# rgoldade/GeometricMultigridPressureSolver

Hardware: AMD Instinct MI355X
Metric: V-cycles/sec (higher is better)
Workload: dtype f32

## Files before the change

### geometricmultigridpressuresolver_amd/csrc/mgps_kernels.hip

```cpp
#include <hip/hip_runtime.h>
#include <hip/hip_fp16.h>

#include <algorithm>
#include <cstdlib>
#include <type_traits>

#include "mgps_internal.h"

namespace mgps {

namespace {

typedef float v4f __attribute__((ext_vector_type(4)));
typedef unsigned char v4b __attribute__((ext_vector_type(4)));
__device__ __forceinline__ float4 streamLoad4(const float *p)
{
    const v4f v = __builtin_nontemporal_load(reinterpret_cast<const v4f *>(p));
    return make_float4(v.x, v.y, v.z, v.w);
}
__device__ __forceinline__ uchar4 streamLoad4(const uint8_t *p)
{
    const v4b v = __builtin_nontemporal_load(reinterpret_cast<const v4b *>(p));
    return make_uchar4(v.x, v.y, v.z, v.w);
}
// ... 516 lines not shown
        const float xs[6] = {me[-1], xc.x, xc.y, xc.z, xc.w, me[4]};
        const float yms[4] = {ym.x, ym.y, ym.z, ym.w}, yps[4] = {yp.x, yp.y, yp.z, yp.w};
        const float zms[4] = {xm.x, xm.y, xm.z, xm.w}, zps[4] = {xp.x, xp.y, xp.z, xp.w};
        const float bs[4] = {bc.x, bc.y, bc.z, bc.w};
        const unsigned ls[4] = {lc.x, lc.y, lc.z, lc.w};
        float res[4];
#pragma unroll
        for (int e = 0; e < 4; ++e) {
            const float diag = simpleDiag(ls[e]);
            const float lap = diag * xs[e + 1] - (xs[e] + xs[e + 2] + yms[e] + yps[e] + zms[e] + zps[e]);
            res[e] = simpleCell(ls[e]) ? epilogueRcp<OP_JACOBI>(xs[e + 1], bs[e], lap, simpleRcp(diag), omega) : inactiveValue<OP_JACOBI>(xs[e + 1]);
        }
        if (valid) gStore4nt(scalarBase(out + ptrdiff_t(k) * sz), opq(off), make_float4(res[0], res[1], res[2], res[3]));
        xc = xp;
        xp = xq;
        hy = hyn;
        hx = hxn;
        lc = lcn;
        lcn = lcq;
        buf ^= 1;
    }
}

__global__ __launch_bounds__(64 * kPlaneRows, 8) void residualZKernel(GridP g, float *__restrict__ rz, const float *__restrict__ x,
                                                                     const float *__restrict__ b, unsigned nbx, unsigned nby, int zc,
                                                                     const int32_t *__restrict__ blocks, const float *__restrict__ rEdge)
{
    __shared__ float plane[2][(kPlaneRows + 2) * kPlanePitch];
    unsigned bid = remapBlock(blockIdx.x, gridDim.x);
    if (blocks) bid = unsigned(blocks[bid]);
    bid = __builtin_amdgcn_readfirstlane(bid);
    const unsigned bx = bid % nbx, by = (bid / nbx) % nby, bz = bid / (nbx * nby);
    const int lane = threadIdx.x & (kWave - 1), ty = threadIdx.x / kWave;
    const int i = int(bx) * 256 + lane * 4, j = int(by) * kPlaneRows + ty;
    const int ic = min(i, g.nx - 4), jc = min(j, g.ny - 1);
    const bool live = ic >= g.xlo && ic < g.xhi;
    const bool valid = i < g.nx && j < g.ny && live;
    const size_t sz = size_t(g.nx) * g.ny;
    const int k0 = int(bz) * zc, k1 = min(k0 + zc, g.nz);
    const int ks = max(k0 - 1, 0), ke = min(k1, g.nz - 1);
    const unsigned offL = unsigned(jc) * unsigned(g.nx) + unsigned(min(max(ic, g.xlo), max(g.xhi - 4, g.xlo)));
    const bool rowTop = ty == 0, rowBot = ty == kPlaneRows - 1, colL = lane == 0, colR = lane == kWave - 1;
    const bool hasL = ic > 0, hasR = ic + 4 < g.nx;
    const int kLo = g.ghostLo ? -1 : 0, kHi = g.ghostHi ? g.nz : g.nz - 1;
    auto planeOf = [&](const float *p, int k) { return scalarBase(p + ptrdiff_t(min(max(k, kLo), kHi)) * ptrdiff_t(sz)); };
    float *const mine0 = plane[0] + (ty + 1) * kPlanePitch + 4 + lane * 4;
    constexpr int kBufFloats = (kPlaneRows + 2) * kPlanePitch;
    const unsigned offHy = (rowTop && jc > 0) ? offL - unsigned(g.nx) : (rowBot && jc < g.ny - 1) ? offL + unsigned(g.nx) : offL;
    {
        const float4 xm = gLoad4(planeOf(x, ks - 1), offL);
        *reinterpret_cast<float4 *>(mine0 + kBufFloats) = keepIf(xm, live);
    }
    const float *xk = planeOf(x, ks);
    float4 xc = gLoad4(xk, offL);
    float4 xp = gLoad4(planeOf(x, ks + 1), offL);
    float4 hy = gLoad4(xk, offHy);
    const bool useHx = live && ((colL && hasL) || (colR && hasR));
    const unsigned offHx = !useHx ? offL : colL ? offL - 1u : offL + 4u;
    float hx = gLoad1(xk, offHx);
    constexpr float w0 = 0.125f, w1 = 0.375f, w2 = 0.375f, w3 = 0.125f;
    float accPrev[4] = {0.f, 0.f, 0.f, 0.f}, accCur[4] = {0.f, 0.f, 0.f, 0.f};
    if (rEdge && k0 == 0 && g.ghostLo) {
        const float4 e = gLoad4(scalarBase(rEdge - ptrdiff_t(sz)), offL);
        accCur[0] = w0 * e.x;
        accCur[1] = w0 * e.y;
        accCur[2] = w0 * e.z;
        accCur[3] = w0 * e.w;
    }
    int buf = 0;
    for (int k = ks; k <= ke; ++k) {
        float *me = mine0 + buf * kBufFloats;
        xc = keepIf(xc, live);
        *reinterpret_cast<float4 *>(me) = xc;
        if (rowTop) *reinterpret_cast<float4 *>(me - kPlanePitch) = keepIf(hy, live);
        if (rowBot) *reinterpret_cast<float4 *>(me + kPlanePitch) = keepIf(hy, live);
        if (colL) me[-1] = useHx ? hx : 0.f;
        if (colR) me[4] = useHx ? hx : 0.f;
        const float *bk = planeOf(b, k);
        const uint8_t *lk = scalarBase(g.lab + size_t(k) * sz);
        const float *xn = planeOf(x, k + 1), *xq2 = planeOf(x, k + 2);
        const float4 bc = gLoad4nt(bk, offL);
        const uchar4 lc = gLoadCodes4nt(lk, offL);
        const float hxn = gLoad1(xn, offHx);
        float4 hyn = hy;
        if (rowTop || rowBot) hyn = gLoad4(xn, offHy);
        const float4 xq = gLoad4(xq2, offL);
        __syncthreads();
        const float4 ym = *reinterpret_cast<const float4 *>(me - kPlanePitch);
        const float4 yp = *reinterpret_cast<const float4 *>(me + kPlanePitch);
        const float4 xm = *reinterpret_cast<const float4 *>(mine0 + (buf ^ 1) * kBufFloats);
        const float xs[6] = {me[-1], xc.x, xc.y, xc.z, xc.w, me[4]};
        const float yms[4] = {ym.x, ym.y, ym.z, ym.w}, yps[4] = {yp.x, yp.y, yp.z, yp.w};
        const float zms[4] = {xm.x, xm.y, xm.z, xm.w}, zps[4] = {xp.x, xp.y, xp.z, xp.w};
        const float bs[4] = {bc.x, bc.y, bc.z, bc.w};
        const unsigned ls[4] = {lc.x, lc.y, lc.z, lc.w};
        float res[4];
#pragma unroll
        for (int e = 0; e < 4; ++e) {
            const float diag = simpleDiag(ls[e]);
            const float lap = diag * xs[e + 1] - (xs[e] + xs[e + 2] + yms[e] + yps[e] + zms[e] + zps[e]);
            res[e] = simpleCell(ls[e]) ? epilogueRcp<OP_RESIDUAL>(xs[e + 1], bs[e], lap, simpleRcp(diag), 0.f) : inactiveValue<OP_RESIDUAL>(xs[e + 1]);
        }
        if (k & 1) {
#pragma unroll
            for (int e = 0; e < 4; ++e) {
                accPrev[e] = accCur[e] + w2 * res[e];
                accCur[e] = w0 * res[e];
            }
        } else {
#pragma unroll
            for (int e = 0; e < 4; ++e) {
                accPrev[e] += w3 * res[e];
                accCur[e] += w1 * res[e];
            }
            if (valid && k >= k0 + 2) gStore4nt(scalarBase(rz + size_t((k >> 1) - 1) * sz), offL, make_float4(accPrev[0], accPrev[1], accPrev[2], accPrev[3]));
        }
        xc = xp;
        xp = xq;
        hy = hyn;
        hx = hxn;
        buf ^= 1;
    }
    if (valid && k1 == g.nz) {
        if (rEdge && g.ghostHi) {
            const float4 e = gLoad4(scalarBase(rEdge + ptrdiff_t(g.nz) * ptrdiff_t(sz)), offL);
            accPrev[0] += w3 * e.x;
            accPrev[1] += w3 * e.y;
            accPrev[2] += w3 * e.z;
            accPrev[3] += w3 * e.w;
        }
        gStore4(rz + size_t((g.nz >> 1) - 1) * sz, offL, make_float4(accPrev[0], accPrev[1], accPrev[2], accPrev[3]));
    }
}

__global__ __launch_bounds__(64 * kPlaneRows) void residualZEdgeKernel(GridP g, float *__restrict__ rz, const float *__restrict__ x, const float *__restrict__ b,
                                                                      unsigned nbx, unsigned nby, int zc, const int32_t *__restrict__ edges)
{
    const unsigned bid = unsigned(edges[blockIdx.x]) >> 1, side = unsigned(edges[blockIdx.x]) & 1u;
    const unsigned bx = bid % nbx, by = (bid / nbx) % nby, bz = bid / (nbx * nby);
    const int k0 = int(bz) * zc, k1 = min(k0 + zc, g.nz);
    const int k = side == 0 ? k0 - 1 : k1, K = side == 0 ? (k0 >> 1) : (k1 >> 1) - 1;
    const float wz = 0.125f;
    if (k < 0 || k >= g.nz) return;
    const int lane = threadIdx.x & (kWave - 1), ty = threadIdx.x / kWave;
    const int i = int(bx) * 256 + lane * 4, j = int(by) * kPlaneRows + ty;
    if (i >= g.nx || j >= g.ny) return;
    const bool live = i >= g.xlo && i < g.xhi;
    const size_t sy = size_t(g.nx), sz = size_t(g.nx) * g.ny;
    const size_t c = size_t(k) * sz + size_t(j) * sy + i;
    const float4 zero4 = make_float4(0.f, 0.f, 0.f, 0.f);
    const size_t cym = j > 0 ? c - sy : c, cyp = j < g.ny - 1 ? c + sy : c, czm = k > 0 ? c - sz : c, czp = k < g.nz - 1 ? c + sz : c;
    const float4 xc = live ? *reinterpret_cast<const float4 *>(x + c) : zero4;
    const float4 ym = live ? *reinterpret_cast<const float4 *>(x + cym) : zero4, yp = live ? *reinterpret_cast<const float4 *>(x + cyp) : zero4;
    const float4 zm = live ? *reinterpret_cast<const float4 *>(x + czm) : zero4, zp = live ? *reinterpret_cast<const float4 *>(x + czp) : zero4;
    const float4 bc = live ? *reinterpret_cast<const float4 *>(b + c) : zero4;
    const unsigned labw = live ? *reinterpret_cast<const unsigned *>(g.lab + c) : 0x01010101u * unsigned(MGPS_EXTERIOR_CELL);
    float left = __shfl_up(xc.w, 1), right = __shfl_down(xc.x, 1);
    if (lane == 0) left = (live && i > 0) ? x[c - 1] : 0.f;
    if (lane == kWave - 1 || i + 4 >= g.nx) right = (live && i + 4 < g.nx) ? x[c + 4] : 0.f;
    if (!live) return;
    const float xs[6] = {left, xc.x, xc.y, xc.z, xc.w, right};
    const float yms[4] = {ym.x, ym.y, ym.z, ym.w}, yps[4] = {yp.x, yp.y, yp.z, yp.w};
    const float zms[4] = {zm.x, zm.y, zm.z, zm.w}, zps[4] = {zp.x, zp.y, zp.z, zp.w};
    const float bs[4] = {bc.x, bc.y, bc.z, bc.w};
    const unsigned ls[4] = {labw & 255u, (labw >> 8) & 255u, (labw >> 16) & 255u, labw >> 24};
    float res[4];
#pragma unroll
    for (int e = 0; e < 4; ++e) {
        const float diag = simpleDiag(ls[e]);
        const float lap = diag * xs[e + 1] - (xs[e] + xs[e + 2] + yms[e] + yps[e] + zms[e] + zps[e]);
        const float r = simpleCell(ls[e]) ? epilogueRcp<OP_RESIDUAL>(xs[e + 1], bs[e], lap, simpleRcp(diag), 0.f) : inactiveValue<OP_RESIDUAL>(xs[e + 1]);
        res[e] = wz * r;
    }
    *reinterpret_cast<float4 *>(rz + size_t(K) * sz + size_t(j) * sy + i) = make_float4(res[0], res[1], res[2], res[3]);
}

template <int OP, bool DOT = false>
__global__ void stencilScalarKernel(GridP g, float *__restrict__ out, const float *__restrict__ x,
                                    const float *__restrict__ b, float omega, double *__restrict__ dotPartials = nullptr)
{
    const size_t n = size_t(g.nx) * g.ny * g.nz;
    const size_t c = size_t(blockIdx.x) * blockDim.x + threadIdx.x;
    double acc = 0.0;
    if (c < n) {
        const unsigned l = g.lab[c];
        const float xc = x[c];
        if (!simpleCell(l)) out[c] = inactiveValue<OP>(xc);
        else {
            const size_t sy = size_t(g.nx), sz = size_t(g.nx) * g.ny;
            const float diag = simpleDiag(l);
            const float lap = diag * xc - (x[c - 1] + x[c + 1] + x[c - sy] + x[c + sy] + x[c - sz] + x[c + sz]);
            const float bc = OP == OP_APPLY ? 0.f : b[c];
            const float res = epilogueRcp<OP>(xc, bc, lap, simpleRcp(diag), omega);
            out[c] = res;
            acc = dotTerm<OP>(xc, bc, res);
        }
    }
    if (DOT) blockDotStore(acc, dotPartials, blockIdx.x);
}

template <int OP, bool DOT = false, class TX = float>
__global__ void boundaryOpKernel(GridP g, TX *__restrict__ out, const TX *__restrict__ x,
                                 const float *__restrict__ b, float omega, unsigned nblocks, double *__restrict__ dotPartials = nullptr,
                                 MixScale ms = MixScale{})
{
    constexpr bool kMixed = !std::is_same<TX, float>::value;
    const unsigned block = remapBlock(blockIdx.x, nblocks);
    const int t = int(block * blockDim.x + threadIdx.x);
    double acc = 0.0;
    if (t < g.nbnd) {
        const size_t c = size_t(g.bnd[t]);
        float lap, diag;
        boundaryRow(g, [&](size_t p) { return Cell<TX>::load1(x + p); }, t, c, lap, diag);
        const float xc = Cell<TX>::load1(x + c), bc = OP == OP_APPLY ? 0.f : b[c];
        float res;
        if (kMixed) {
            const float bm = mixRhsScale(ms);
            res = OP == OP_JACOBI ? xc + omega * ((bm * bc - lap) / diag) : OP == OP_RESIDUAL ? bm * bc - ms.c2 * lap : lap;
        } else
            res = epilogue<OP>(xc, bc, lap, diag, omega);
        Cell<TX>::store1(out + c, res);
        acc = dotTerm<OP>(xc, bc, kMixed ? __half2float(toHalfSat(res)) : res);
    }
    if (DOT) blockDotStore(acc, dotPartials, blockIdx.x);
}

__global__ void bandComputeKernel(GridP g, const float *__restrict__ x, const float *__restrict__ b,
                                  const int32_t *__restrict__ band, int nband, float *__restrict__ tmp, float omega,
                                  unsigned nblocks)
{
    const unsigned block = remapBlock(blockIdx.x, nblocks);
    const int t = int(block * blockDim.x + threadIdx.x);
    if (t >= nband) return;
    const size_t c = size_t(band[t]);
    const size_t sy = size_t(g.nx), sz = size_t(g.nx) * g.ny;
    const float xc = x[c];
    float lap, diag;
    if (t >= g.nbnd) {
        diag = float(g.bandDiag[t]);
        lap = diag * xc - (x[c - 1] + x[c + 1] + x[c - sy] + x[c + sy] + x[c - sz] + x[c + sz]);
        tmp[t] = xc + omega * ((b[c] - lap) * simpleRcp(diag));
    } else {
        boundaryRow(g, [&](size_t p) { return x[p]; }, t, c, lap, diag);
        tmp[t] = xc + omega * ((b[c] - lap) / diag);
    }
}
template <bool DOT = false, class TX = float>
__global__ void bandScatterKernel(TX *__restrict__ x, const int32_t *__restrict__ band, int nband,
                                  const float *__restrict__ tmp, unsigned nblocks, const float *__restrict__ b = nullptr,
                                  double *__restrict__ dotPartials = nullptr)
{
    const int t = int(remapBlock(blockIdx.x, nblocks) * blockDim.x + threadIdx.x);
    double acc = 0.0;
    if (t < nband) {
        const int32_t c = band[t];
        const float v = tmp[t];
        if (DOT) {
            const float stored = std::is_same<TX, float>::value ? v : __half2float(toHalfSat(v));
            acc = (double(stored) - double(Cell<TX>::load1(x + c))) * double(b[c]);
        }
        Cell<TX>::store1(x + c, v);
    }
    if (DOT) blockDotStore(acc, dotPartials, blockIdx.x);
}

__device__ __forceinline__ bool boxBand(unsigned cls) { return cls >= kBoxGeneral && cls <= kBoxSimple + 6; }

template <class TX, bool CLOSURE, bool DOT, bool GEN, bool XZERO, bool PRO = false>
__device__ __forceinline__ void bandBoxBody(const GridP &g, const TX *__restrict__ src, const float *__restrict__ b, TX *dst,
                                            TX *__restrict__ snap, const int32_t *__restrict__ info, const uint32_t *__restrict__ list,
                                            const int32_t *__restrict__ general, float omega, int depth, const MixScale &ms,
                                            double *__restrict__ dotPartials, const TX *dotOld, int outClosure, unsigned group, unsigned slot,
                                            const float *__restrict__ coarse = nullptr)
{
    static_assert(!PRO || (CLOSURE && !XZERO && std::is_same<TX, float>::value), "the prolonged input: closure mode, fp32");
    constexpr bool kMixed = !std::is_same<TX, float>::value;
    constexpr int kGenRows = GEN ? kBoxMaxGeneral : 1;
    __shared__ __attribute__((aligned(16))) float val[2][kBoxMaxNodes];
    __shared__ float grow[7][kGenRows];
    __shared__ float gbv[kGenRows];
    __shared__ uint16_t gnode[kGenRows], gring[kGenRows];
    const int32_t *gip = info + kBoxInfoInts * size_t(group);
    int gi[kBoxInfoInts];
#pragma unroll
    for (int q = 0; q < kBoxInfoInts; ++q) gi[q] = __builtin_amdgcn_readfirstlane(gip[q]);
    const int rx = gi[1] & 255, ry = (gi[1] >> 8) & 255, sxy = rx * ry;
    const unsigned sy = unsigned(g.nx), sz = unsigned(g.nx) * unsigned(g.ny);
    const ptrdiff_t origin = gi[0];
    if (!XZERO) src += origin;
    b += origin;
    if (dst) dst += origin;
    if (CLOSURE && snap) snap += origin;
    if (DOT) dotOld += origin;
    const uint32_t *U = list + gi[2];
    const int ngen = GEN ? gi[5] : 0, nList = CLOSURE ? gi[7] : gi[3];
    const int H = depth + (CLOSURE ? 1 : 0);
    const float bm = kMixed ? mixRhsScale(ms) : 1.f;
    const int tid = threadIdx.x;
    auto nodeOf = [&](uint32_t e) { return int(__umul24((e >> 10) & 31u, unsigned(sxy)) + __umul24((e >> 5) & 31u, unsigned(rx)) + (e & 31u)); };
    auto cellOf = [&](uint32_t e) { return (e & 31u) + __umul24((e >> 5) & 31u, sy) + __umul24((e >> 10) & 31u, sz); };
    auto rd = [&](const TX *base, unsigned c) { return Cell<TX>::load1(reinterpret_cast<const TX *>(reinterpret_cast<const char *>(base) + c * unsigned(sizeof(TX)))); };
    auto rdf = [&](const float *base, unsigned c) { return *reinterpret_cast<const float *>(reinterpret_cast<const char *>(base) + c * 4u); };
    auto wr = [&](TX *base, unsigned c, float v) { Cell<TX>::store1(reinterpret_cast<TX *>(reinterpret_cast<char *>(base) + c * unsigned(sizeof(TX))), v); };
    uint32_t ue[kBoxSlots];
    float bv[kBoxSlots];
    {
#pragma unroll
        for (int m = 0; m < kBoxSlots; ++m) {
            const int k = tid + m * kBoxThreads;
            ue[m] = k < nList ? U[k] : (uint32_t(kBoxSkip) << 16);
        }
        uint32_t ge = 0;
        int32_t grw = 0;
        if (GEN && tid < ngen) {
            ge = uint32_t(general[2 * size_t(gi[4] + tid)]);
            grw = general[2 * size_t(gi[4] + tid) + 1];
        }
        float xv[kBoxSlots];
#pragma unroll
        for (int m = 0; m < kBoxSlots; ++m) {
            const unsigned cls = (ue[m] >> 16) & 15u;
            const bool need = cls != kBoxSkip && cls != kBoxZero && (CLOSURE || cls != kBoxFrozenFar);
            const bool bneed = (cls > kBoxSimple && cls <= kBoxSimple + 6 && int(ue[m] >> 20) <= H - 1) || (CLOSURE && cls == kBoxFrozenOut);
            const unsigned c = cellOf(ue[m]);
            xv[m] = XZERO ? 0.f : rd(src, need ? c : 0u);
            bv[m] = rdf(b, bneed ? c : 0u);
        }
#pragma unroll
        for (int m = 0; m < kBoxSlots; ++m) {
            const unsigned cls = (ue[m] >> 16) & 15u;
            if (cls == kBoxSkip || cls == kBoxZero) xv[m] = 0.f;
            if (kMixed) bv[m] *= bm;
        }
        {
            const int rz = (gi[1] >> 16) & 255, ncell4 = (sxy * rz + 3) >> 2;
            float4 *z0 = reinterpret_cast<float4 *>(val[0]), *z1 = reinterpret_cast<float4 *>(val[1]);
            for (int q = tid; q < ncell4; q += kBoxThreads) {
                z0[q] = make_float4(0.f, 0.f, 0.f, 0.f);
                z1[q] = make_float4(0.f, 0.f, 0.f, 0.f);
            }
        }
        __syncthreads();
        if (GEN && tid < ngen) {
            const uint32_t e = ge;
            gring[tid] = uint16_t(e >> 20);
            gnode[tid] = uint16_t(nodeOf(e));
            const size_t nb = size_t(g.nbnd);
#pragma unroll
            for (int q = 0; q < 7; ++q) grow[q][tid] = g.rows[size_t(q) * nb + grw];
            const unsigned c = cellOf(e);
            gbv[tid] = kMixed ? bm * rdf(b, c) : rdf(b, c);
        }
#pragma unroll
        for (int m = 0; m < kBoxSlots; ++m)
            if (tid + m * kBoxThreads < nList) {
                const int n = nodeOf(ue[m]);
                val[0][n] = xv[m];
                val[1][n] = xv[m];
            }
    }
    __syncthreads();
    if (PRO) {
        const int ox = int(origin % g.nx), oy = int((origin / g.nx) % g.ny), oz = int(origin / sz);
        const int cnx = g.nx >> 1, cny = g.ny >> 1, cnz = g.nz >> 1;
        const unsigned csy = unsigned(cnx), csz = unsigned(cnx) * unsigned(cny);
        const float *cb = scalarBase(coarse);
#pragma unroll
        for (int m = 0; m < kBoxSlots; ++m) {
            if (m > 0) asm volatile("" ::: "memory");
            const uint32_t e = ue[m];
            const unsigned cls = (e >> 16) & 15u;
            if (tid + m * kBoxThreads < nList && cls != kBoxSkip && cls != kBoxZero) {
                const int ci = ox + int(e & 31u), cj = oy + int((e >> 5) & 31u), ck = oz + int((e >> 10) & 31u);
                const int bi = min(max((ci - 1) >> 1, 0), cnx - 2), bj = min(max((cj - 1) >> 1, 0), cny - 2), bk = min(max((ck - 1) >> 1, 0), cnz - 2);
                const float fx = (ci & 1) ? 0.25f : 0.75f, fy = (cj & 1) ? 0.25f : 0.75f, fz = (ck & 1) ? 0.25f : 0.75f;
                const unsigned o = unsigned(bk) * csz + unsigned(bj) * csy + unsigned(bi);
                const float v00 = lerpRef(gLoad1(cb, o), gLoad1(cb, o + 1u), fx), v10 = lerpRef(gLoad1(cb, o + csy), gLoad1(cb, o + csy + 1u), fx);
                const float v01 = lerpRef(gLoad1(cb, o + csz), gLoad1(cb, o + csz + 1u), fx), v11 = lerpRef(gLoad1(cb, o + csz + csy), gLoad1(cb, o + csz + csy + 1u), fx);
                const int n = nodeOf(e);
                const float v = val[0][n] + 4.f * lerpRef(lerpRef(v00, v10, fy), lerpRef(v01, v11, fy), fz);
                val[0][n] = v;
                val[1][n] = v;
            }
        }
        __syncthreads();
    }
    for (int p = 1; p <= H; ++p) {
        const float *from = val[(p - 1) & 1];
        float *to = val[p & 1];
        const int lim = H - p;
        const bool last = CLOSURE && p == H;
#pragma unroll
        for (int m = 0; m < kBoxSlots; ++m) {
            const unsigned cls = (ue[m] >> 16) & 15u;
            const bool simple = cls > kBoxSimple && cls <= kBoxSimple + 6;
            if ((simple && int(ue[m] >> 20) <= lim) || (last && cls == kBoxFrozenOut)) {
                const int n = nodeOf(ue[m]);
                const float xc = from[n];
                const float diag = cls == kBoxFrozenOut ? 6.f : float(int(cls) - int(kBoxSimple));
                const float lap = diag * xc - (from[n - 1] + from[n + 1] + from[n - rx] + from[n + rx] + from[n - sxy] + from[n + sxy]);
                to[n] = xc + omega * ((bv[m] - lap) * simpleRcp(diag));
            }
        }
        if (GEN && tid < ngen && int(gring[tid]) <= lim) {
            const int nd = gnode[tid];
            const float xc = from[nd];
            float acc = 0.f;
            acc -= grow[0][tid] * from[nd - 1];
            acc -= grow[1][tid] * from[nd + 1];
            acc -= grow[2][tid] * from[nd - rx];
            acc -= grow[3][tid] * from[nd + rx];
            acc -= grow[4][tid] * from[nd - sxy];
            acc -= grow[5][tid] * from[nd + sxy];
            const float diag = grow[6][tid];
            const float lap = acc + diag * xc;
            to[nd] = xc + omega * ((gbv[tid] - lap) / diag);
        }
        __syncthreads();
    }
    const float *fin = val[H & 1];
    double acc = 0.0;
#pragma unroll
    for (int m = 0; m < kBoxSlots; ++m) {
        const unsigned cls = (ue[m] >> 16) & 15u;
        if ((ue[m] >> 20) == 0u && (boxBand(cls) || ((CLOSURE || outClosure) && cls == kBoxFrozenOut))) {
            const unsigned c = cellOf(ue[m]);
            const float v = fin[nodeOf(ue[m])];
            if (DOT) {
                const float stored = kMixed ? __half2float(toHalfSat(v)) : v;
                acc += (double(stored) - double(rd(dotOld, c))) * double(rdf(b, c));
            }
            if (dst) wr(dst, c, v);
            if (CLOSURE && snap) wr(snap, c, v);
        }
    }
    if (DOT) blockDotStore(acc, dotPartials, slot);
}
template <class TX, bool CLOSURE, bool DOT, bool GEN, bool XZERO = false, bool PRO = false>
__global__ __launch_bounds__(kBoxThreads, 8) void bandBoxKernel(GridP g, const TX *__restrict__ src, const float *__restrict__ b, TX *dst,
                                                              TX *__restrict__ snap, const int32_t *__restrict__ info, const uint32_t *__restrict__ list,
                                                              const int32_t *__restrict__ general, float omega, int depth, MixScale ms,
                                                              double *__restrict__ dotPartials, const TX *dotOld, int outClosure,
                                                              const float *__restrict__ coarse = nullptr)
{
    bandBoxBody<TX, CLOSURE, DOT, GEN, XZERO, PRO>(g, src, b, dst, snap, info, list, general, omega, depth, ms, dotPartials, dotOld, outClosure,
                                                   remapBlock(blockIdx.x, gridDim.x), blockIdx.x, coarse);
}

template <bool GEN, bool XZERO>
__global__ __launch_bounds__(kBoxThreads, 8) void strokeFrontKernel(GridP g, float *__restrict__ out, const float *__restrict__ x, const float *__restrict__ b,
                                                                  float *__restrict__ snap, const int32_t *__restrict__ info, const uint32_t *__restrict__ list,
                                                                  const int32_t *__restrict__ general, float omega, int depth, unsigned ngroups,
                                                                  unsigned nshares, const int32_t *__restrict__ chunks, const uint32_t *__restrict__ keep)
{
    if (blockIdx.x < ngroups) {
        bandBoxBody<float, true, false, GEN, XZERO>(g, x, b, nullptr, snap, info, list, general, omega, depth, MixScale{}, nullptr, nullptr, 0,
                                                    remapBlock(blockIdx.x, ngroups), 0u);
        return;
    }
    const unsigned share = (blockIdx.x - ngroups) * (kBoxThreads / 256) + (threadIdx.x >> 8);
    if (share < nshares) stencilQuadBody<OP_JACOBI, false, float, XZERO, true>(g, out, x, b, omega, nshares, chunks, nullptr, MixScale{}, share, threadIdx.x & 255u, keep);
}
__global__ __launch_bounds__(256) void markClosureKernel(GridP g, const int32_t *__restrict__ info, const uint32_t *__restrict__ list, uint32_t *__restrict__ bits)
{
    const int32_t *gi = info + kBoxInfoInts * size_t(blockIdx.x);
    const size_t sy = size_t(g.nx), sz = size_t(g.nx) * g.ny, origin = size_t(gi[0]);
    const uint32_t *U = list + gi[2];
    for (int k = threadIdx.x; k < gi[7]; k += 256) {
        const uint32_t e = U[k];
        const unsigned cls = (e >> 16) & 15u;
        if ((e >> 20) != 0u || !(boxBand(cls) || cls == kBoxFrozenOut)) continue;
        const size_t c = origin + (e & 31u) + ((e >> 5) & 31u) * sy + ((e >> 10) & 31u) * sz;
        atomicOr(bits + (c >> 5), 1u << (c & 31));
    }
}

__global__ __launch_bounds__(256) void markSnapTilesKernel(GridP g, const int32_t *__restrict__ info, const uint32_t *__restrict__ list, uint8_t *__restrict__ tiles)
{
    const int32_t *gi = info + kBoxInfoInts * size_t(blockIdx.x);
    const int tx = (g.nx + kTile - 1) / kTile, ty = (g.ny + kTile - 1) / kTile;
    const size_t origin = size_t(gi[0]);
    const int ox = int(origin % size_t(g.nx)), oy = int((origin / size_t(g.nx)) % size_t(g.ny)), oz = int(origin / (size_t(g.nx) * g.ny));
    const uint32_t *U = list + gi[2];
    for (int k = threadIdx.x; k < gi[7]; k += 256) {
        const uint32_t e = U[k];
        const unsigned cls = (e >> 16) & 15u;
        if (cls == kBoxSkip || cls == kBoxZero) continue;
        const int i = ox + int(e & 31u), j = oy + int((e >> 5) & 31u), k3 = oz + int((e >> 10) & 31u);
        tiles[(size_t(k3 / kTile) * ty + j / kTile) * tx + i / kTile] = 1;
    }
}

template <class TX>
__global__ __launch_bounds__(kBoxThreads) void bandBoxCopyKernel(GridP g, const TX *__restrict__ src, TX *__restrict__ dst, const int32_t *__restrict__ info,
                                                                const uint32_t *__restrict__ list)
{
    const int32_t *gi = info + kBoxInfoInts * size_t(remapBlock(blockIdx.x, gridDim.x));
    const ptrdiff_t sy = g.nx, sz = ptrdiff_t(g.nx) * g.ny, origin = gi[0];
    const uint32_t *U = list + gi[2];
    for (int k = threadIdx.x; k < gi[7]; k += kBoxThreads) {
        const uint32_t e = U[k];
        if ((e >> 20) != 0u || !boxBand((e >> 16) & 15u)) continue;
        const ptrdiff_t c = origin + ptrdiff_t(e & 31u) + ptrdiff_t((e >> 5) & 31u) * sy + ptrdiff_t((e >> 10) & 31u) * sz;
        dst[c] = src[c];
    }
}

constexpr int kHalo = kTile + 2;
constexpr int kHalo3 = kHalo * kHalo * kHalo;
constexpr int kTile3 = kTile * kTile * kTile;
constexpr int kPlanes = 3 * (kTile - 1) + 1;
constexpr int kRowPool = 240;

__device__ __forceinline__ int haloIdx(int li, int lj, int lk) { return ((lk + 1) * kHalo + (lj + 1)) * kHalo + (li + 1); }

template <bool LABELS, class TX = float>
__device__ __forceinline__ void gsLoadTile(const GridP &g, const TX *__restrict__ x, const float *__restrict__ b,
                                           int i0, int j0, int k0, float *sx, float *sb, unsigned char *sl, float bm = 1.f)
{
    constexpr bool kMixed = !std::is_same<TX, float>::value;
    const bool full = i0 + kTile <= g.nx && j0 + kTile <= g.ny && k0 + kTile <= g.nz;
    if (full) {
        const int tid = threadIdx.x;
        float4 xv[6], bv[4];
        uchar4 lv[6];
        float hv[3];
        unsigned char hl[3];
#pragma unroll
        for (int m = 0; m < 6; ++m) {
            const int r = tid + m * 256;
            const int q = r & 3, lj = (r >> 2) % kHalo, lk = (r >> 2) / kHalo;
            const int gj = j0 + lj - 1, gk = k0 + lk - 1;
            const bool in = r < kHalo * kHalo * 4 && gj >= 0 && gk >= -g.ghostLo && gj < g.ny && gk < g.nz + g.ghostHi;
            const ptrdiff_t rowOff = (ptrdiff_t(gk) * g.ny + gj) * g.nx + i0 + 4 * q;
            xv[m] = make_float4(0.f, 0.f, 0.f, 0.f);
            lv[m] = make_uchar4(MGPS_EXTERIOR_CELL, MGPS_EXTERIOR_CELL, MGPS_EXTERIOR_CELL, MGPS_EXTERIOR_CELL);
            if (in) {
                xv[m] = Cell<TX>::load4(x + rowOff);
                if (LABELS && lj >= 1 && lj <= kTile && lk >= 1 && lk <= kTile) lv[m] = *reinterpret_cast<const uchar4 *>(g.lab + rowOff);
            }
        }
#pragma unroll
        for (int m = 0; m < 3; ++m) {
            const int r = tid + m * 256;
            const int side = r & 1, lj = (r >> 1) % kHalo, lk = (r >> 1) / kHalo;
            const int gi = side ? i0 + kTile : i0 - 1, gj = j0 + lj - 1, gk = k0 + lk - 1;
            const bool in = r < kHalo * kHalo * 2 && gi >= 0 && gi < g.nx && gj >= 0 && gk >= -g.ghostLo && gj < g.ny && gk < g.nz + g.ghostHi;
            const ptrdiff_t c = (ptrdiff_t(gk) * g.ny + gj) * g.nx + gi;
            hv[m] = 0.f;
            hl[m] = (unsigned char)MGPS_EXTERIOR_CELL;
            if (in) hv[m] = Cell<TX>::load1(x + c);
        }
#pragma unroll
        for (int m = 0; m < 4; ++m) {
            const int r = tid + m * 256;
            const int q = r & 3, lj = (r >> 2) % kTile, lk = (r >> 2) / kTile;
            bv[m] = g.streaming ? streamLoad4(b + (size_t(k0 + lk) * g.ny + j0 + lj) * g.nx + i0 + 4 * q)
                                : *reinterpret_cast<const float4 *>(b + (size_t(k0 + lk) * g.ny + j0 + lj) * g.nx + i0 + 4 * q);
        }
#pragma unroll
        for (int m = 0; m < 6; ++m) {
            const int r = tid + m * 256;
            if (r < kHalo * kHalo * 4) {
                const int at = (r >> 2) * kHalo + 1 + 4 * (r & 3);
                sx[at] = xv[m].x;
                sx[at + 1] = xv[m].y;
                sx[at + 2] = xv[m].z;
                sx[at + 3] = xv[m].w;
                if (LABELS) {
                    sl[at] = lv[m].x;
                    sl[at + 1] = lv[m].y;
                    sl[at + 2] = lv[m].z;
                    sl[at + 3] = lv[m].w;
                }
            }
        }
#pragma unroll
        for (int m = 0; m < 3; ++m) {
            const int r = tid + m * 256;
            if (r < kHalo * kHalo * 2) {
                const int h = (r >> 1) * kHalo + ((r & 1) ? kHalo - 1 : 0);
                sx[h] = hv[m];
                if (LABELS) sl[h] = hl[m];
            }
        }
#pragma unroll
        for (int m = 0; m < 4; ++m) {
            float *dst = sb + (tid + m * 256) * 4;
            dst[0] = kMixed ? bm * bv[m].x : bv[m].x;
            dst[1] = kMixed ? bm * bv[m].y : bv[m].y;
            dst[2] = kMixed ? bm * bv[m].z : bv[m].z;
            dst[3] = kMixed ? bm * bv[m].w : bv[m].w;
        }
    } else {
        for (int h = threadIdx.x; h < kHalo3; h += blockDim.x) {
            const int li = h % kHalo, lj = (h / kHalo) % kHalo, lk = h / (kHalo * kHalo);
            const int gi = i0 + li - 1, gj = j0 + lj - 1, gk = k0 + lk - 1;
            const bool in = gi >= 0 && gj >= 0 && gk >= -g.ghostLo && gi < g.nx && gj < g.ny && gk < g.nz + g.ghostHi;
            const ptrdiff_t c = in ? (ptrdiff_t(gk) * g.ny + gj) * g.nx + gi : 0;
            sx[h] = in ? Cell<TX>::load1(x + c) : 0.f;
            if (LABELS) sl[h] = in ? g.lab[c] : (unsigned char)MGPS_EXTERIOR_CELL;
        }
        for (int h = threadIdx.x; h < kTile3; h += blockDim.x) {
            const int li = h % kTile, lj = (h / kTile) % kTile, lk = h / (kTile * kTile);
            const int gi = i0 + li, gj = j0 + lj, gk = k0 + lk;
            const bool in = gi < g.nx && gj < g.ny && gk < g.nz;
            sb[h] = in ? (kMixed ? bm * b[(size_t(gk) * g.ny + gj) * g.nx + gi] : b[(size_t(gk) * g.ny + gj) * g.nx + gi]) : 0.f;
        }
    }
}

template <bool DOT, class TX = float>
__device__ __forceinline__ void gsPureTile(const GridP &g, TX *__restrict__ x, const float *__restrict__ b, int tile, int forward,
                                           double *__restrict__ dotPartials, unsigned slot, float *sx, float *sb, float bm = 1.f,
                                           TX *__restrict__ snap = nullptr, const uint8_t *__restrict__ snapTile = nullptr)
{
    const int tilesX = (g.nx + kTile - 1) / kTile, tilesY = (g.ny + kTile - 1) / kTile;
    const int i0 = (tile % tilesX) * kTile, j0 = ((tile / tilesX) % tilesY) * kTile, k0 = (tile / (tilesX * tilesY)) * kTile;
    gsLoadTile<false, TX>(g, x, b, i0, j0, k0, sx, sb, nullptr, bm);
    __syncthreads();
    const int li = threadIdx.x % kTile, lj = threadIdx.x / kTile;
    for (int step = 0; step < kPlanes; ++step) {
        const int s = forward ? step : kPlanes - 1 - step;
        const int lk = s - li - lj;
        if (lk >= 0 && lk < kTile) {
            const int h = haloIdx(li, lj, lk);
            const float xc = sx[h];
            const float lap = 6.f * xc - (sx[h - 1] + sx[h + 1] + sx[h - kHalo] + sx[h + kHalo] + sx[h - kHalo * kHalo] +
                                          sx[h + kHalo * kHalo]);
            sx[h] = xc + (sb[(lk * kTile + lj) * kTile + li] - lap) * (1.f / 6.f);
        }
        __syncthreads();
    }
    double acc = 0.0;
    const bool snapOn = snap && snapTile[tile];
    for (int r = threadIdx.x; r < kTile * kTile * 4; r += blockDim.x) {
        const int q = r & 3, cj = (r >> 2) % kTile, ck = (r >> 2) / kTile;
        const float *src = sx + haloIdx(4 * q, cj, ck);
        const size_t at = (size_t(k0 + ck) * g.ny + j0 + cj) * g.nx + i0 + 4 * q;
        Cell<TX>::store4(x + at, make_float4(src[0], src[1], src[2], src[3]));
        if (snapOn) Cell<TX>::store4(snap + at, make_float4(src[0], src[1], src[2], src[3]));
        if (DOT) {
            const float *bq = sb + (ck * kTile + cj) * kTile + 4 * q;
#pragma unroll
            for (int e = 0; e < 4; ++e) acc += double(src[e]) * double(bq[e]);
        }
    }
    if (DOT) blockDotStore(acc, dotPartials, slot);
}
template <bool DOT = false, class TX = float>
__global__ __launch_bounds__(256) void tiledGSPureKernel(GridP g, TX *__restrict__ x, const float *__restrict__ b,
                                                         const int32_t *__restrict__ tiles, int forward,
                                                         double *__restrict__ dotPartials = nullptr, MixScale ms = MixScale{},
                                                         TX *__restrict__ snap = nullptr, const uint8_t *__restrict__ snapTile = nullptr)
{
    __shared__ float sx[kHalo3];
    __shared__ float sb[kTile3];
    const unsigned bid = remapBlock(blockIdx.x, gridDim.x);
    gsPureTile<DOT, TX>(g, x, b, tiles[bid], forward, dotPartials, bid, sx, sb, std::is_same<TX, float>::value ? 1.f : mixRhsScale(ms), snap, snapTile);
}

template <bool DOT, class TX = float>
__device__ __forceinline__ void gsMixedTile(const GridP &g, TX *__restrict__ x, const float *__restrict__ b, int tile,
                                            const int32_t *__restrict__ tileBndStart, int forward, double *__restrict__ dotPartials,
                                            unsigned slot, float *sx, float *sb, unsigned char *sl, float *srow, unsigned short *rowMask,
                                            unsigned short *rowStart, int *scanTmp, float bm = 1.f, TX *__restrict__ snap = nullptr,
                                            const uint8_t *__restrict__ snapTile = nullptr)
{
    const int tilesX = (g.nx + kTile - 1) / kTile, tilesY = (g.ny + kTile - 1) / kTile;
    const int i0 = (tile % tilesX) * kTile, j0 = ((tile / tilesX) % tilesY) * kTile, k0 = (tile / (tilesX * tilesY)) * kTile;
    const int bndBase = tileBndStart[tile], bndCount = tileBndStart[tile + 1] - bndBase;
    const size_t nb = size_t(g.nbnd);
    gsLoadTile<true, TX>(g, x, b, i0, j0, k0, sx, sb, sl, bm);
    for (int r = threadIdx.x; r < 7 * min(bndCount, kRowPool); r += blockDim.x) {
        const int q = r / min(bndCount, kRowPool), t = r % min(bndCount, kRowPool);
        srow[q * kRowPool + t] = g.rows[q * nb + bndBase + t];
    }
    __syncthreads();
    if (bndCount > 0) {
        const int rj = threadIdx.x % kTile, rk = threadIdx.x / kTile;
        unsigned m = 0;
        for (int i = 0; i < kTile; ++i) m |= (sl[haloIdx(i, rj, rk)] == kCodeGeneral) ? (1u << i) : 0u;
        rowMask[threadIdx.x] = (unsigned short)m;
        int cnt = __popc(m), incl = cnt;
        const int lane = threadIdx.x & (kWave - 1), wave = threadIdx.x / kWave;
#pragma unroll
        for (int off = 1; off < kWave; off <<= 1) {
            const int v = __shfl_up(incl, off);
            if (lane >= off) incl += v;
// ... 2260 lines not shown
```

Measured before the change: 116.6.

## Stage coarse prolongation window in shared memory before fine-box interpolation

In the prolongation-fused box smoother, the block now loads the coarse-grid window covering its box once, cooperatively and coalesced, into the second shared buffer. Each node then reads its eight trilinear neighbours from that buffer instead of making eight scattered global loads. The coarse loads are issued early so they overlap with the list and RHS loads. In exchange the code adds extra barriers and a second zeroing pass of the buffer, and it assumes the coarse window fits in 18^3 cells.

```diff
diff --git a/geometricmultigridpressuresolver_amd/csrc/mgps_kernels.hip b/geometricmultigridpressuresolver_amd/csrc/mgps_kernels.hip
--- a/geometricmultigridpressuresolver_amd/csrc/mgps_kernels.hip
+++ b/geometricmultigridpressuresolver_amd/csrc/mgps_kernels.hip
@@ -842,6 +842,19 @@
     auto rd = [&](const TX *base, unsigned c) { return Cell<TX>::load1(reinterpret_cast<const TX *>(reinterpret_cast<const char *>(base) + c * unsigned(sizeof(TX)))); };
     auto rdf = [&](const float *base, unsigned c) { return *reinterpret_cast<const float *>(reinterpret_cast<const char *>(base) + c * 4u); };
     auto wr = [&](TX *base, unsigned c, float v) { Cell<TX>::store1(reinterpret_cast<TX *>(reinterpret_cast<char *>(base) + c * unsigned(sizeof(TX))), v); };
+    constexpr int kBoxCoarseSlots = (18 * 18 * 18 + kBoxThreads - 1) / kBoxThreads;
+    int ox = 0, oy = 0, oz = 0, cnx = 0, cny = 0, cnz = 0, cx0 = 0, cy0 = 0, cz0 = 0, cwx = 1, cwxy = 1, ncoarse = 0;
+    unsigned csy = 0, csz = 0;
+    if (PRO) {
+        ox = int(origin % g.nx), oy = int((origin / g.nx) % g.ny), oz = int(origin / sz);
+        cnx = g.nx >> 1, cny = g.ny >> 1, cnz = g.nz >> 1;
+        csy = unsigned(cnx), csz = unsigned(cnx) * unsigned(cny);
+        const int rz = (gi[1] >> 16) & 255;
+        cx0 = min(max((ox - 1) >> 1, 0), cnx - 2), cy0 = min(max((oy - 1) >> 1, 0), cny - 2), cz0 = min(max((oz - 1) >> 1, 0), cnz - 2);
+        cwx = min(max((ox + rx - 2) >> 1, 0), cnx - 2) + 2 - cx0;
+        const int cwy = min(max((oy + ry - 2) >> 1, 0), cny - 2) + 2 - cy0, cwz = min(max((oz + rz - 2) >> 1, 0), cnz - 2) + 2 - cz0;
+        cwxy = cwx * cwy, ncoarse = cwxy * cwz;
+    }
     uint32_t ue[kBoxSlots];
     float bv[kBoxSlots];
     {
@@ -855,6 +868,21 @@
         if (GEN && tid < ngen) {
             ge = uint32_t(general[2 * size_t(gi[4] + tid)]);
             grw = general[2 * size_t(gi[4] + tid) + 1];
+        }
+        if (PRO) {
+            const float rXY = 1.f / float(cwxy), rX = 1.f / float(cwx);
+            const float *cb = scalarBase(coarse + (size_t(cz0) * csz + size_t(cy0) * csy + size_t(cx0)));
+            float cv[kBoxCoarseSlots];
+#pragma unroll
+            for (int m = 0; m < kBoxCoarseSlots; ++m) {
+                const int q = tid + m * kBoxThreads;
+                const int z = int((float(q) + 0.5f) * rXY), r = q - z * cwxy;
+                const int y = int((float(r) + 0.5f) * rX), x = r - y * cwx;
+                cv[m] = gLoad1(cb, q < ncoarse ? unsigned(z) * csz + unsigned(y) * csy + unsigned(x) : 0u);
+            }
+#pragma unroll
+            for (int m = 0; m < kBoxCoarseSlots; ++m)
+                if (tid + m * kBoxThreads < ncoarse) val[1][tid + m * kBoxThreads] = cv[m];
         }
         float xv[kBoxSlots];
 #pragma unroll
@@ -877,7 +905,7 @@
             float4 *z0 = reinterpret_cast<float4 *>(val[0]), *z1 = reinterpret_cast<float4 *>(val[1]);
             for (int q = tid; q < ncell4; q += kBoxThreads) {
                 z0[q] = make_float4(0.f, 0.f, 0.f, 0.f);
-                z1[q] = make_float4(0.f, 0.f, 0.f, 0.f);
+                if (!PRO) z1[q] = make_float4(0.f, 0.f, 0.f, 0.f);
             }
         }
         __syncthreads();
@@ -891,40 +919,37 @@
             const unsigned c = cellOf(e);
             gbv[tid] = kMixed ? bm * rdf(b, c) : rdf(b, c);
         }
+        if (PRO) {
+#pragma unroll
+            for (int m = 0; m < kBoxSlots; ++m) {
+                const uint32_t e = ue[m];
+                const unsigned cls = (e >> 16) & 15u;
+                if (tid + m * kBoxThreads < nList && cls != kBoxSkip && cls != kBoxZero) {
+                    const int ci = ox + int(e & 31u), cj = oy + int((e >> 5) & 31u), ck = oz + int((e >> 10) & 31u);
+                    const int bi = min(max((ci - 1) >> 1, 0), cnx - 2), bj = min(max((cj - 1) >> 1, 0), cny - 2), bk = min(max((ck - 1) >> 1, 0), cnz - 2);
+                    const float fx = (ci & 1) ? 0.25f : 0.75f, fy = (cj & 1) ? 0.25f : 0.75f, fz = (ck & 1) ? 0.25f : 0.75f;
+                    const float *cw = val[1] + ((bk - cz0) * cwxy + (bj - cy0) * cwx + (bi - cx0));
+                    const float v00 = lerpRef(cw[0], cw[1], fx), v10 = lerpRef(cw[cwx], cw[cwx + 1], fx);
+                    const float v01 = lerpRef(cw[cwxy], cw[cwxy + 1], fx), v11 = lerpRef(cw[cwxy + cwx], cw[cwxy + cwx + 1], fx);
+                    xv[m] += 4.f * lerpRef(lerpRef(v00, v10, fy), lerpRef(v01, v11, fy), fz);
+                }
+                if (tid + m * kBoxThreads < nList) val[0][nodeOf(e)] = xv[m];
+            }
+            __syncthreads();
+            const int rz = (gi[1] >> 16) & 255, ncell4 = (sxy * rz + 3) >> 2;
+            float4 *z1 = reinterpret_cast<float4 *>(val[1]);
+            for (int q = tid; q < ncell4; q += kBoxThreads) z1[q] = make_float4(0.f, 0.f, 0.f, 0.f);
+            __syncthreads();
+        }
 #pragma unroll
         for (int m = 0; m < kBoxSlots; ++m)
             if (tid + m * kBoxThreads < nList) {
                 const int n = nodeOf(ue[m]);
-                val[0][n] = xv[m];
+                if (!PRO) val[0][n] = xv[m];
                 val[1][n] = xv[m];
             }
     }
     __syncthreads();
-    if (PRO) {
-        const int ox = int(origin % g.nx), oy = int((origin / g.nx) % g.ny), oz = int(origin / sz);
-        const int cnx = g.nx >> 1, cny = g.ny >> 1, cnz = g.nz >> 1;
-        const unsigned csy = unsigned(cnx), csz = unsigned(cnx) * unsigned(cny);
-        const float *cb = scalarBase(coarse);
-#pragma unroll
-        for (int m = 0; m < kBoxSlots; ++m) {
-            if (m > 0) asm volatile("" ::: "memory");
-            const uint32_t e = ue[m];
-            const unsigned cls = (e >> 16) & 15u;
-            if (tid + m * kBoxThreads < nList && cls != kBoxSkip && cls != kBoxZero) {
-                const int ci = ox + int(e & 31u), cj = oy + int((e >> 5) & 31u), ck = oz + int((e >> 10) & 31u);
-                const int bi = min(max((ci - 1) >> 1, 0), cnx - 2), bj = min(max((cj - 1) >> 1, 0), cny - 2), bk = min(max((ck - 1) >> 1, 0), cnz - 2);
-                const float fx = (ci & 1) ? 0.25f : 0.75f, fy = (cj & 1) ? 0.25f : 0.75f, fz = (ck & 1) ? 0.25f : 0.75f;
-                const unsigned o = unsigned(bk) * csz + unsigned(bj) * csy + unsigned(bi);
-                const float v00 = lerpRef(gLoad1(cb, o), gLoad1(cb, o + 1u), fx), v10 = lerpRef(gLoad1(cb, o + csy), gLoad1(cb, o + csy + 1u), fx);
-                const float v01 = lerpRef(gLoad1(cb, o + csz), gLoad1(cb, o + csz + 1u), fx), v11 = lerpRef(gLoad1(cb, o + csz + csy), gLoad1(cb, o + csz + csy + 1u), fx);
-                const int n = nodeOf(e);
-                const float v = val[0][n] + 4.f * lerpRef(lerpRef(v00, v10, fy), lerpRef(v01, v11, fy), fz);
-                val[0][n] = v;
-                val[1][n] = v;
-            }
-        }
-        __syncthreads();
-    }
     for (int p = 1; p <= H; ++p) {
         const float *from = val[(p - 1) & 1];
         float *to = val[p & 1];
```

New measurement: 115.4. Within noise of the previous version (-1.0%).
